# google-research/seed_rl

Hardware: NVIDIA H100
Metric: env-frames/sec (learner, device-timed) on synthetic 84x84x4 T=20 unrolls @1/2/4/8 H100 (higher is better)
Workload: dtype bf16x3 (fp32-faithful tensor-core contraction; activations stored as bf16 hi+lo pairs), f32 elsewhere

## Files before the change

### seed_rl_b200/csrc/conv_planes.cu

```cuda
#include <cuda.h>
#include <cuda_bf16.h>

#include <cstdio>
#include <cstdlib>

#include "kernels.h"
#include "tc_common.cuh"

namespace seedrl {

long long planes_positions(int N, int H, int W) {
  const long long Q = (long long)N * (H + 1) * (W + 2);
  return ((Q + 2 * (W + 2) + 2 + 256 + 127) / 128) * 128;
}
size_t planes_bytes(int N, int H, int W, int C) {
  return (size_t)planes_positions(N, H, W) * 16 * 2 * (C / 8);
}

typedef CUresult (*EncodeTiledFn)(CUtensorMap*, CUtensorMapDataType, cuuint32_t, void*, const cuuint64_t*,
                                  const cuuint64_t*, const cuuint32_t*, const cuuint32_t*,
                                  CUtensorMapInterleave, CUtensorMapSwizzle, CUtensorMapL2promotion,
                                  CUtensorMapFloatOOBfill);
static EncodeTiledFn encode_tiled_fn() {
  static EncodeTiledFn fn = nullptr;
  static bool tried = false;
  if (!tried) {
    tried = true;
    void* q = nullptr;
    cudaDriverEntryPointQueryResult qr;
    if (cudaGetDriverEntryPoint("cuTensorMapEncodeTiled", &q, cudaEnableDefault, &qr) == cudaSuccess &&
        qr == cudaDriverEntryPointSuccess)
      fn = reinterpret_cast<EncodeTiledFn>(q);
    (void)cudaGetLastError();
  }
  return fn;
}

static int g_chunk = 0;
int planes_chunk() {
  if (g_chunk == 0) {
    const char* e = getenv("SEEDRL_PLANES_CHUNK");
    g_chunk = e ? atoi(e) : 128;
    if (g_chunk != 16 && g_chunk != 32 && g_chunk != 64 && g_chunk != 128) g_chunk = 128;
  }
  return g_chunk;
}

static int make_plane_map(CUtensorMap* tm, const void* base, long long Lp, int planes, int shift,
                          int CH, int box_chunks, int box_planes) {
  EncodeTiledFn enc = encode_tiled_fn();
  if (!enc) return set_error(SEEDRL_ERR_INTERNAL, "cuTensorMapEncodeTiled is not available");
  if (box_chunks < 1 || box_chunks > 256 || box_planes < 1 || box_planes > planes)
    return set_error(SEEDRL_ERR_INVALID_ARGUMENT, "conv planes: TMA box out of range");
  const cuuint64_t gdim[3] = {(cuuint64_t)(2 * CH), (cuuint64_t)((Lp - shift) / CH), (cuuint64_t)planes};
  const cuuint64_t gstr[2] = {(cuuint64_t)CH * 16, (cuuint64_t)Lp * 16};
  const cuuint32_t box[3] = {(cuuint32_t)(2 * CH), (cuuint32_t)box_chunks, (cuuint32_t)box_planes};
  const cuuint32_t estr[3] = {1, 1, 1};
  void* addr = const_cast<char*>(reinterpret_cast<const char*>(base)) + (size_t)shift * 16;
  const CUresult r = enc(tm, CU_TENSOR_MAP_DATA_TYPE_UINT64, 3, addr, gdim, gstr, box, estr,
                         CU_TENSOR_MAP_INTERLEAVE_NONE, CU_TENSOR_MAP_SWIZZLE_NONE,
                         CU_TENSOR_MAP_L2_PROMOTION_L2_256B, CU_TENSOR_MAP_FLOAT_OOB_FILL_NONE);
  if (r != CUDA_SUCCESS) {
    char msg[128];
    snprintf(msg, sizeof msg, "cuTensorMapEncodeTiled failed (%d) Lp=%lld planes=%d shift=%d box=%dx%d", (int)r, Lp,
             planes, shift, box_chunks, box_planes);
    return set_error(SEEDRL_ERR_INTERNAL, msg);
  }
  return SEEDRL_OK;
}

__device__ __forceinline__ void mbar_expect_tx(uint64_t* bar, uint32_t bytes) {
  asm volatile("mbarrier.arrive.expect_tx.shared::cta.b64 _, [%0], %1;" ::"r"(smem_u32(bar)), "r"(bytes)
               : "memory");
}
__device__ __forceinline__ void tma_load_3d(void* dst, const CUtensorMap* tm, int c0, int c1, int c2,
                                            uint64_t* bar) {
  asm volatile(
      "cp.async.bulk.tensor.3d.shared::cluster.global.tile.mbarrier::complete_tx::bytes [%0], [%1, {%2, %3, %4}], [%5];" ::
          "r"(smem_u32(dst)),
      "l"(reinterpret_cast<uint64_t>(tm)), "r"(c0), "r"(c1), "r"(c2), "r"(smem_u32(bar))
      : "memory");
}
__device__ __forceinline__ float bf16lo(uint32_t w) { return __uint_as_float(w << 16); }
__device__ __forceinline__ float bf16hi(uint32_t w) { return __uint_as_float(w & 0xFFFF0000u); }

struct ConvpArgs {
  ConvGeom g;
  int Lp;
  int nch;
  int chunk;
  int ntiles;
  int nb;
  const uint4* wq;
  const float* bias;
  const uint4* mask;
  const uint4* res;
  uint4* out_raw;
  uint4* out_relu;
  float* out_nhwc;
  int* err;
};

constexpr int kCpWarpgroups = 4;
constexpr int kCpThreads = 128 * kCpWarpgroups + 32;
constexpr int kCpM = 128;
constexpr int kCpMaxStages = 4;

__device__ __forceinline__ void quad_transpose(float2 (&t)[4], int q) {
#pragma unroll
  for (int b = 1; b <= 2; b <<= 1) {
    const bool up = (q & b) != 0;
#pragma unroll
    for (int u = 0; u < 4; ++u) {
      if (u & b) continue;
      const float2 send = up ? t[u] : t[u | b];
      const float2 r = make_float2(__shfl_xor_sync(0xffffffffu, send.x, b), __shfl_xor_sync(0xffffffffu, send.y, b));
      if (up) t[u] = r; else t[u | b] = r;
    }
  }
}

template <int CIN, int COUT, int NSUB>
__global__ void __launch_bounds__(kCpThreads, 1)
convp_kernel(const __grid_constant__ CUtensorMap tm_in, const ConvpArgs a) {
  constexpr int G = CIN / 8, GO = COUT / 8, NS = CIN / 16;
  constexpr int MT = NSUB * kCpM;
  constexpr int NBLK = 2 * NSUB;
  extern __shared__ __align__(128) uint8_t smem_raw[];
  const int PW = a.g.PW, nb = a.nb;
  const uint32_t P = (uint32_t)(a.nch * a.chunk) * 16u;
  const uint32_t stage_bytes = 2u * G * P;
  uint8_t* s_stage = smem_raw;
  uint4* s_b = reinterpret_cast<uint4*>(smem_raw + (size_t)nb * stage_bytes);
  float* s_bias = reinterpret_cast<float*>(s_b + 2 * 9 * CIN * COUT / 8);
  uint64_t* s_full = reinterpret_cast<uint64_t*>(s_bias + COUT);
  uint64_t* s_empty = s_full + kCpMaxStages;
  const int tid = threadIdx.x, warp = tid >> 5, lane = tid & 31;

  for (int i = tid; i < 2 * 9 * CIN * COUT / 8; i += kCpThreads) s_b[i] = __ldg(a.wq + i);
  if (tid < COUT) s_bias[tid] = a.bias ? __ldg(a.bias + tid) : 0.f;
  if (tid == 0) {
    for (int i = 0; i < nb; ++i) {
      mbar_init(s_full + i, 1);
      mbar_init(s_empty + i, 4 * kCpWarpgroups);
    }
    asm volatile("fence.mbarrier_init.release.cluster;" ::: "memory");
    asm volatile("prefetch.tensormap [%0];" ::"l"(reinterpret_cast<uint64_t>(&tm_in)) : "memory");
  }
  asm volatile("fence.proxy.async.shared::cta;" ::: "memory");
  __syncthreads();

  const int my_tiles = ((int)blockIdx.x < a.ntiles) ? (a.ntiles - 1 - (int)blockIdx.x) / (int)gridDim.x + 1 : 0;
  bool timed_out = false;

  if (warp == 4 * kCpWarpgroups) {
    if (elect_one()) {
      for (int it = 0; it < my_tiles; ++it) {
        const int s = it % nb;
        if (it >= nb && !mbar_wait_bounded(s_empty + s, (uint32_t)(((it / nb) - 1) & 1))) { timed_out = true; break; }
        const int tile = (int)blockIdx.x + it * (int)gridDim.x;
        mbar_expect_tx(s_full + s, stage_bytes);
        tma_load_3d(s_stage + (size_t)s * stage_bytes, &tm_in, 0, tile * MT / a.chunk, 0, s_full + s);
      }
    }
    __syncwarp();
  } else {
    const int cw = warp >> 2;
    const size_t plane_u = (size_t)a.Lp;
    if (blockIdx.x == 0) {
      const uint4 z = make_uint4(0u, 0u, 0u, 0u);
      for (int i = tid; i < (PW + 1) * 2 * GO; i += 128 * kCpWarpgroups) {
        const int pl = i / (PW + 1), s = i - pl * (PW + 1);
        if (a.out_raw) a.out_raw[(size_t)pl * plane_u + s] = z;
        if (a.out_relu) a.out_relu[(size_t)pl * plane_u + s] = z;
      }
    }
    const int q = lane & 3;
    const int row = 16 * (warp & 3) + (lane >> 2) + 8 * (q & 1);
    const uint32_t b_base = smem_u32(s_b);
    const uint64_t db0 = gmma_desc(b_base, (uint32_t)(2 * GO) * 128u, 128u);
    for (int it = 0; it < my_tiles; ++it) {
      const int s = it % nb;
      const int tile = (int)blockIdx.x + it * (int)gridDim.x;
      if (!mbar_wait_bounded(s_full + s, (uint32_t)((it / nb) & 1))) { timed_out = true; break; }
      const int m0 = (cw - it * NBLK) & (kCpWarpgroups - 1);
      if (m0 >= NBLK && lane == 0) mbar_arrive(s_empty + s);
      const uint32_t a_base = smem_u32(s_stage + (size_t)s * stage_bytes);
      const uint64_t da0 = gmma_desc(a_base, P, 128u);
      const uint64_t lo_off = (uint64_t)((G * P) >> 4), slab_off = (uint64_t)((2 * P) >> 4);
#pragma unroll 1
      for (int m = m0; m < NBLK; m += kCpWarpgroups) {
        float acc[COUT];
#pragma unroll
        for (int i = 0; i < COUT; ++i) acc[i] = 0.f;
        wgmma_fence_acc<COUT>(acc);
        wgmma_fence();
#pragma unroll
        for (int tap = 0; tap < 9; ++tap) {
          const uint64_t off = (uint64_t)(m * 64 + (tap / 3) * PW + (tap % 3));
#pragma unroll
          for (int sl = 0; sl < NS; ++sl) {
            const uint64_t da = da0 + off + (uint64_t)sl * slab_off;
            const uint64_t db = db0 + (uint64_t)((tap * NS + sl) * (COUT * 64 / 16));
            Wgmma<2 * COUT>::template mma<0, 0>(acc, da, db, 1u);
            Wgmma<COUT>::template mma<0, 0>(acc, da + lo_off, db, 1u);
          }
        }
        wgmma_commit();
        const int p = tile * MT + m * 64 + row;
        const int sp = p + PW + 1;
        const int pix = out_pixel(a.g, p);
        uint4 mk[GO / 2], rh[GO / 2], rl[GO / 2];
        if (pix >= 0) {
#pragma unroll
          for (int k = 0; k < GO / 2; ++k) {
            const int go = (q >> 1) + 2 * k;
            if (a.mask) mk[k] = __ldg(a.mask + (size_t)go * plane_u + sp);
            if (a.res) {
              rh[k] = __ldg(a.res + (size_t)go * plane_u + sp);
              rl[k] = __ldg(a.res + (size_t)(GO + go) * plane_u + sp);
            }
          }
        }
        wgmma_wait<0>();
        wgmma_fence_acc<COUT>(acc);
        if (m + kCpWarpgroups >= NBLK && lane == 0) mbar_arrive(s_empty + s);
        const bool in_store = sp < a.Lp;
#pragma unroll
        for (int k = 0; k < GO / 2; ++k) {
          const int go = (q >> 1) + 2 * k;
          float2 t[4];
#pragma unroll
          for (int u = 0; u < 4; ++u) {
            const int j = 2 * k + (u >> 1), h = u & 1;
            t[u] = make_float2(acc[4 * j + 2 * h] + acc[4 * (j + GO) + 2 * h],
                               acc[4 * j + 2 * h + 1] + acc[4 * (j + GO) + 2 * h + 1]);
          }
          quad_transpose(t, q);
          float x[8];
#pragma unroll
          for (int e = 0; e < 4; ++e) {
            x[2 * e] = t[e].x + s_bias[go * 8 + 2 * e];
            x[2 * e + 1] = t[e].y + s_bias[go * 8 + 2 * e + 1];
          }
          if (pix >= 0 && a.mask) {
            const uint32_t mw[4] = {mk[k].x, mk[k].y, mk[k].z, mk[k].w};
#pragma unroll
            for (int e = 0; e < 4; ++e) {
              x[2 * e] = bf16lo(mw[e]) > 0.f ? x[2 * e] : 0.f;
              x[2 * e + 1] = bf16hi(mw[e]) > 0.f ? x[2 * e + 1] : 0.f;
            }
          }
          if (pix >= 0 && a.res) {
            const uint32_t hw[4] = {rh[k].x, rh[k].y, rh[k].z, rh[k].w};
            const uint32_t lw[4] = {rl[k].x, rl[k].y, rl[k].z, rl[k].w};
#pragma unroll
            for (int e = 0; e < 4; ++e) {
              x[2 * e] += bf16lo(hw[e]) + bf16lo(lw[e]);
              x[2 * e + 1] += bf16hi(hw[e]) + bf16hi(lw[e]);
            }
          }
          if (pix < 0) {
#pragma unroll
            for (int e = 0; e < 8; ++e) x[e] = 0.f;
          }
          const float4 xa = make_float4(x[0], x[1], x[2], x[3]), xb = make_float4(x[4], x[5], x[6], x[7]);
          if (a.out_raw && in_store) {
            a.out_raw[(size_t)go * plane_u + sp] = pack8_bf16(xa, xb);
            a.out_raw[(size_t)(GO + go) * plane_u + sp] = pack8_bf16(bf16_resid4(xa), bf16_resid4(xb));
          }
          if (a.out_relu && in_store) {
            const float4 ra = make_float4(fmaxf(xa.x, 0.f), fmaxf(xa.y, 0.f), fmaxf(xa.z, 0.f), fmaxf(xa.w, 0.f));
            const float4 rb = make_float4(fmaxf(xb.x, 0.f), fmaxf(xb.y, 0.f), fmaxf(xb.z, 0.f), fmaxf(xb.w, 0.f));
            a.out_relu[(size_t)go * plane_u + sp] = pack8_bf16(ra, rb);
            a.out_relu[(size_t)(GO + go) * plane_u + sp] = pack8_bf16(bf16_resid4(ra), bf16_resid4(rb));
          }
          if (a.out_nhwc && pix >= 0) {
            float4* o = reinterpret_cast<float4*>(a.out_nhwc + (size_t)pix * COUT + go * 8);
            o[0] = xa; o[1] = xb;
          }
        }
      }
    }
  }
  if (timed_out && a.err) atomicExch(a.err, 1);
}

template <int CIN, int COUT, int NSUB>
static int launch_convp(const PlaneConv& c, cudaStream_t st) {
  const ConvGeom g = make_geom(c.N, c.H, c.W);
  constexpr int MT = NSUB * kCpM;
  const long long Lp = planes_positions(c.N, c.H, c.W);
  if (Lp + MT + 4 * g.PW >= (1LL << 31))
    return set_error(SEEDRL_ERR_INVALID_ARGUMENT, "convp: batch too large for 32-bit positions");
  const int L = MT + 2 * g.PW + 2;
  const int CH = planes_chunk();
  const int nch = (L + CH - 1) / CH;
  const size_t stage = (size_t)2 * (CIN / 8) * nch * CH * 16;
  const size_t fixed = (size_t)2 * 9 * CIN * COUT * 2 + COUT * 4 + 2 * kCpMaxStages * 8;
  int nb = kCpMaxStages;
  while (nb > 1 && nb * stage + fixed > 227 * 1024) --nb;
  if (nb < 2) return kPlanesTryNext;
  const size_t smem = nb * stage + fixed;
  CUtensorMap tm;
  SEEDRL_TRY(make_plane_map(&tm, c.in, Lp, 2 * (CIN / 8), 0, CH, nch, 2 * (CIN / 8)));
  static bool attr = false;
  if (!attr) {
    SEEDRL_CUDA(cudaFuncSetAttribute(convp_kernel<CIN, COUT, NSUB>, cudaFuncAttributeMaxDynamicSharedMemorySize,
                                     227 * 1024));
    attr = true;
  }
  ConvpArgs a;
  a.g = g; a.Lp = (int)Lp; a.nch = nch; a.chunk = CH; a.nb = nb;
  a.ntiles = (int)((Lp - g.PW - 1 + MT - 1) / MT);
  a.wq = reinterpret_cast<const uint4*>(c.wq); a.bias = c.bias;
  a.mask = reinterpret_cast<const uint4*>(c.mask); a.res = reinterpret_cast<const uint4*>(c.res);
  a.out_raw = reinterpret_cast<uint4*>(c.out_raw); a.out_relu = reinterpret_cast<uint4*>(c.out_relu);
  a.out_nhwc = c.out_nhwc; a.err = c.err;
  const int grid = a.ntiles < kNumSMs ? a.ntiles : kNumSMs;
  convp_kernel<CIN, COUT, NSUB><<<grid, kCpThreads, smem, st>>>(tm, a);
  count_launch(g_conv_cat, st);
  SEEDRL_CHECK_LAUNCH();
  return SEEDRL_OK;
}

bool convp_supported(int cin, int cout) {
  return (cin == 16 || cin == 32) && (cout == 16 || cout == 32);
}

int convp_forward(int cin, int cout, const PlaneConv& c, cudaStream_t st) {
  const long long Lp = planes_positions(c.N, c.H, c.W);
  const bool small = Lp / 512 < 2 * kNumSMs;
#define SEEDRL_CP_CASE(CI, CO_)                                                   \
  if (cin == CI && cout == CO_) {                                                 \
    int rc = kPlanesTryNext;                                                      \
    if (!small) rc = launch_convp<CI, CO_, 4>(c, st);                             \
    if (rc == kPlanesTryNext) rc = launch_convp<CI, CO_, 2>(c, st);               \
    if (rc == kPlanesTryNext) rc = launch_convp<CI, CO_, 1>(c, st);               \
    if (rc == kPlanesTryNext) return set_error(SEEDRL_ERR_INVALID_ARGUMENT, "convp: image too wide"); \
    return rc;                                                                    \
  }
  SEEDRL_CP_CASE(16, 16)
  SEEDRL_CP_CASE(16, 32)
  SEEDRL_CP_CASE(32, 16)
  SEEDRL_CP_CASE(32, 32)
#undef SEEDRL_CP_CASE
  return set_error(SEEDRL_ERR_INVALID_ARGUMENT, "convp: unsupported (cin,cout)");
}

struct WgradpArgs {
  int PW, T, nchunks, nb;
  int chunk;
  float* partial;
  int* err;
};

constexpr int kWpMaxStages = 6;
constexpr int kWpHaloRow = 8;
__host__ __device__ constexpr int wgradp_mtiles(int CP) { return 3 * CP + 1 <= 64 ? 1 : 2; }
__host__ __device__ constexpr int wgradp_khsplit(int CP) { return CP == 16 ? 3 : 1; }
__host__ __device__ constexpr int wgradp_threads(int CP) { return 128 * wgradp_mtiles(CP) * wgradp_khsplit(CP) + 32; }

struct WgradMaps { CUtensorMap x, x_halo, dy, dy_halo; };

template <int CP, int COUT, int KC>
__global__ void __launch_bounds__(wgradp_threads(CP), 1)
wgradp_kernel(const __grid_constant__ WgradMaps tm, const WgradpArgs a) {
  constexpr int G = CP / 8, GO = COUT / 8;
  constexpr int MT = wgradp_mtiles(CP), KSPL = wgradp_khsplit(CP), NCW = MT * KSPL;
  constexpr int NKH = 3 / KSPL;
  constexpr int NW = 9 * CP * COUT + COUT;
  constexpr uint32_t Px = (KC + kWpHaloRow) * 16;
  extern __shared__ __align__(128) uint8_t smem_raw[];
  const int nb = a.nb, PW = a.PW;
  const uint32_t Pd = (uint32_t)(KC + a.T) * 16u;
  const uint32_t x_bytes = 2u * G * Px;
  const uint32_t stage_bytes = x_bytes + 2u * GO * Pd;
  uint64_t* s_full = reinterpret_cast<uint64_t*>(smem_raw);
  uint64_t* s_empty = s_full + kWpMaxStages;
  uint8_t* s_stage = smem_raw + 128;
  const int tid = threadIdx.x, warp = tid >> 5, lane = tid & 31;

  if (tid == 0) {
    for (int i = 0; i < kWpMaxStages; ++i) { mbar_init(s_full + i, 1); mbar_init(s_empty + i, 4 * NCW); }
    asm volatile("fence.mbarrier_init.release.cluster;" ::: "memory");
  }
  __syncthreads();

  const int my_chunks = ((int)blockIdx.x < a.nchunks) ? (a.nchunks - 1 - (int)blockIdx.x) / (int)gridDim.x + 1 : 0;
  bool timed_out = false;

  if (warp == 4 * NCW) {
    if (elect_one()) {
      for (int it = 0; it < my_chunks; ++it) {
        const int s = it % nb;
        if (it >= nb && !mbar_wait_bounded(s_empty + s, (uint32_t)(((it / nb) - 1) & 1))) { timed_out = true; break; }
        const int j0 = ((int)blockIdx.x + it * (int)gridDim.x) * KC;
        uint8_t* xs = s_stage + (size_t)s * stage_bytes;
        uint8_t* ds = xs + x_bytes;
        mbar_expect_tx(s_full + s, stage_bytes);
        for (int p = 0; p < 2 * G; ++p) {
          tma_load_3d(xs + p * Px, &tm.x, 0, j0 / a.chunk, p, s_full + s);
          tma_load_3d(xs + p * Px + KC * 16, &tm.x_halo, 0, (j0 + KC) / kWpHaloRow, p, s_full + s);
        }
        for (int p = 0; p < 2 * GO; ++p) {
          tma_load_3d(ds + p * Pd, &tm.dy, 0, j0 / a.chunk, p, s_full + s);
          tma_load_3d(ds + p * Pd + KC * 16, &tm.dy_halo, 0, (j0 + KC) / kWpHaloRow, p, s_full + s);
        }
      }
    }
    __syncwarp();
  } else {
    const int cw = warp >> 2, mt = cw % MT, kh0 = (cw / MT) * NKH;
    const int mg0 = 8 * mt + 2 * (warp & 3);
    const int mg = mg0 + ((lane >> 3) & 1);
    const uint32_t a_off = (mg < 3 * G ? (uint32_t)(mg % G) * Px + (uint32_t)(mg / G) * 16u : 0u) +
                           (uint32_t)((lane >> 4) * 8 + (lane & 7)) * 16u;
    const bool data0 = mg0 < 3 * G, data1 = mg0 + 1 < 3 * G;
    const uint32_t one = (lane >> 2) == 0 ? 0x3F803F80u : 0u;
    const uint32_t c0 = mg0 == 3 * G ? one : 0u, c1 = mg0 + 1 == 3 * G ? one : 0u;
    float acc[NKH][COUT];
#pragma unroll
    for (int i = 0; i < NKH * COUT; ++i) (&acc[0][0])[i] = 0.f;
    wgmma_fence_acc<NKH * COUT>(&acc[0][0]);
    const uint64_t desc0 = gmma_desc(0u, 128u, Pd);
    const uint32_t desc_lo = (uint32_t)desc0, desc_hi = (uint32_t)(desc0 >> 32);
    for (int it = 0; it < my_chunks; ++it) {
      const int s = it % nb;
      if (!mbar_wait_bounded(s_full + s, (uint32_t)((it / nb) & 1))) { timed_out = true; break; }
      const uint32_t sb = smem_u32(s_stage + (size_t)s * stage_bytes);
      const uint32_t xb = sb + a_off;
      const uint32_t db = desc_lo + ((sb + x_bytes) >> 4) + (uint32_t)((2 - kh0) * PW);
      uint32_t ah[2][4], al[2][4];
#pragma unroll
      for (int ks = 0; ks < KC / 16; ++ks) {
        uint32_t(&h)[4] = ah[ks & 1];
        uint32_t(&l)[4] = al[ks & 1];
        ldsm_x4_trans(h, xb + ks * 256);
        ldsm_x4_trans(l, xb + G * Px + ks * 256);
        if (!data0) { h[0] = h[2] = c0; l[0] = l[2] = 0u; }
        if (!data1) { h[1] = h[3] = c1; l[1] = l[3] = 0u; }
        wgmma_fence();
#pragma unroll
        for (int kh = 0; kh < NKH; ++kh) {
          const uint64_t b = make_desc64(db - (uint32_t)(kh * PW) + (uint32_t)(ks * 16), desc_hi);
          WgmmaRA<2 * COUT>::template mma<1>(acc[kh], h, b, 1u);
          WgmmaRA<COUT>::template mma<1>(acc[kh], l, b, 1u);
        }
        wgmma_commit();
        wgmma_wait<1>();
      }
      wgmma_wait<0>();
      if (lane == 0) mbar_arrive(s_empty + s);
    }
    wgmma_fence_acc<NKH * COUT>(&acc[0][0]);
    float* dst = a.partial + (size_t)blockIdx.x * NW;
#pragma unroll
    for (int h = 0; h < 2; ++h) {
      const int row = 64 * mt + 16 * (warp & 3) + (lane >> 2) + 8 * h;
      const int kw = row / CP, ci = row - kw * CP;
#pragma unroll
      for (int k = 0; k < NKH; ++k) {
        const int kh = kh0 + k;
#pragma unroll
        for (int j = 0; j < GO; ++j) {
#pragma unroll
          for (int e = 0; e < 2; ++e) {
            const int co = 8 * j + 2 * (lane & 3) + e;
            const float v = acc[k][4 * j + 2 * h + e] + acc[k][4 * j + 2 * h + e + COUT / 2];
            if (row < 3 * CP) dst[((size_t)(kh * 3 + kw) * CP + ci) * COUT + co] = v;
            else if (row == 3 * CP && kh == 1) dst[9 * CP * COUT + co] = v;
          }
        }
      }
    }
  }
  if (timed_out && a.err) atomicExch(a.err, 1);
}

template <int CP, int COUT, int KC>
static int launch_wgradp(int N, int H, int W, const void* x, const void* dy, float* dw, float* db, int* err,
                         WgradBatch* batch, cudaStream_t st) {
  const ConvGeom g = make_geom(N, H, W);
  const long long Lp = planes_positions(N, H, W);
  constexpr int G = CP / 8, GO = COUT / 8;
  const int CH = planes_chunk() < KC ? planes_chunk() : KC;
  if (KC % CH) return kPlanesTryNext;
  const int T = (2 * g.PW + kWpHaloRow - 1) / kWpHaloRow * kWpHaloRow;
  const size_t stage = (size_t)2 * G * (KC + kWpHaloRow) * 16 + (size_t)2 * GO * (KC + T) * 16;
  int nb = kWpMaxStages;
  while (nb > 1 && 128 + nb * stage > 227 * 1024) --nb;
  if (nb < 2) return kPlanesTryNext;
  const size_t smem = 128 + nb * stage;
  WgradMaps tm;
  SEEDRL_TRY(make_plane_map(&tm.x, x, Lp, 2 * G, g.PW, CH, KC / CH, 1));
  SEEDRL_TRY(make_plane_map(&tm.x_halo, x, Lp, 2 * G, g.PW, kWpHaloRow, 1, 1));
  SEEDRL_TRY(make_plane_map(&tm.dy, dy, Lp, 2 * GO, 1, CH, KC / CH, 1));
  SEEDRL_TRY(make_plane_map(&tm.dy_halo, dy, Lp, 2 * GO, 1, kWpHaloRow, T / kWpHaloRow, 1));
  static bool attr = false;
  if (!attr) {
    SEEDRL_CUDA(cudaFuncSetAttribute(wgradp_kernel<CP, COUT, KC>, cudaFuncAttributeMaxDynamicSharedMemorySize,
                                     227 * 1024));
    attr = true;
  }
  static const bool dbg = getenv("SEEDRL_DEBUG_LAUNCH") != nullptr;
  if (dbg) fprintf(stderr, "wgradp<%d,%d,%d> CH=%d T=%d nb=%d stage=%zu smem=%zu\n", CP, COUT, KC, CH, T, nb, stage, smem);
  constexpr int NW = 9 * CP * COUT + COUT;
  WgradpArgs a;
  a.PW = g.PW; a.T = T; a.nb = nb; a.err = err; a.chunk = CH;
  a.nchunks = (int)((g.Q + g.PW + KC - 1) / KC);
  const int grid = a.nchunks < kNumSMs ? a.nchunks : kNumSMs;
  if (!batch || batch->n >= kMaxReduceJobs || batch->used + (size_t)grid * NW > batch->cap_floats)
    return set_error(SEEDRL_ERR_INVALID_ARGUMENT, "wgradp: partial buffer too small");
  a.partial = batch->buf + batch->used;
  batch->used += (size_t)grid * NW;
  wgradp_kernel<CP, COUT, KC><<<grid, wgradp_threads(CP), smem, st>>>(tm, a);
  count_launch(PC_CONV_WGRAD, st);
  SEEDRL_CHECK_LAUNCH();
  batch->jobs[batch->n++] = ReduceJob{a.partial, dw, db, grid, 9 * CP * COUT, COUT};
  return SEEDRL_OK;
}

int wgradp(int cin, int cout, int N, int H, int W, const void* x, const void* dy, float* dw, float* db,
           int* err, WgradBatch* batch, cudaStream_t st) {
#define SEEDRL_WP_CASE(CI, CO_, KC0)                                                                        \
  if (cin == CI && cout == CO_) {                                                                           \
    int rc = kPlanesTryNext;                                                                                \
    if constexpr (KC0 >= 256) rc = launch_wgradp<CI, CO_, 256>(N, H, W, x, dy, dw, db, err, batch, st);     \
    if (rc == kPlanesTryNext) rc = launch_wgradp<CI, CO_, 128>(N, H, W, x, dy, dw, db, err, batch, st);     \
    if (rc == kPlanesTryNext) rc = launch_wgradp<CI, CO_, 64>(N, H, W, x, dy, dw, db, err, batch, st);      \
    if (rc == kPlanesTryNext) return set_error(SEEDRL_ERR_INVALID_ARGUMENT, "wgradp: does not fit");        \
    return rc;                                                                                              \
  }
  SEEDRL_WP_CASE(16, 16, 256)
  SEEDRL_WP_CASE(16, 32, 128)
  SEEDRL_WP_CASE(32, 32, 128)
#undef SEEDRL_WP_CASE
  return set_error(SEEDRL_ERR_INVALID_ARGUMENT, "wgradp: unsupported (cin,cout)");
}

__global__ void to_planes_kernel(ConvGeom g, int Lp, int G, int relu, const float* __restrict__ x,
                                 uint4* __restrict__ out) {
  const long long i = (long long)blockIdx.x * blockDim.x + threadIdx.x;
  if (i >= (long long)Lp * G) return;
  const int s = (int)(i / G), go = (int)(i - (long long)s * G);
  const int pix = in_pixel(g, s);
  float4 a = make_float4(0.f, 0.f, 0.f, 0.f), b = a;
  if (pix >= 0) {
    const float4* src = reinterpret_cast<const float4*>(x + (size_t)pix * (G * 8) + go * 8);
    a = __ldg(src); b = __ldg(src + 1);
    if (relu) {
      a.x = fmaxf(a.x, 0.f); a.y = fmaxf(a.y, 0.f); a.z = fmaxf(a.z, 0.f); a.w = fmaxf(a.w, 0.f);
      b.x = fmaxf(b.x, 0.f); b.y = fmaxf(b.y, 0.f); b.z = fmaxf(b.z, 0.f); b.w = fmaxf(b.w, 0.f);
    }
  }
  out[(size_t)go * Lp + s] = pack8_bf16(a, b);
  out[(size_t)(G + go) * Lp + s] = pack8_bf16(bf16_resid4(a), bf16_resid4(b));
}

__global__ void from_planes_kernel(ConvGeom g, int Lp, int G, const uint4* __restrict__ in, float* __restrict__ y) {
  const long long i = (long long)blockIdx.x * blockDim.x + threadIdx.x;
  if (i >= (long long)Lp * G) return;
  const int s = (int)(i / G), go = (int)(i - (long long)s * G);
  const int pix = in_pixel(g, s);
  if (pix < 0) return;
  const uint4 h = __ldg(in + (size_t)go * Lp + s), l = __ldg(in + (size_t)(G + go) * Lp + s);
  float4* dst = reinterpret_cast<float4*>(y + (size_t)pix * (G * 8) + go * 8);
  dst[0] = make_float4(bf16lo(h.x) + bf16lo(l.x), bf16hi(h.x) + bf16hi(l.x), bf16lo(h.y) + bf16lo(l.y),
                       bf16hi(h.y) + bf16hi(l.y));
  dst[1] = make_float4(bf16lo(h.z) + bf16lo(l.z), bf16hi(h.z) + bf16hi(l.z), bf16lo(h.w) + bf16lo(l.w),
                       bf16hi(h.w) + bf16hi(l.w));
}

int to_planes(int N, int H, int W, int C, int relu, const float* x, void* out, cudaStream_t st) {
  const ConvGeom g = make_geom(N, H, W);
  const long long Lp = planes_positions(N, H, W);
  const long long n = Lp * (C / 8);
  to_planes_kernel<<<(unsigned)((n + 255) / 256), 256, 0, st>>>(g, (int)Lp, C / 8, relu, x,
                                                                reinterpret_cast<uint4*>(out));
  count_launch(PC_MISC, st);
  SEEDRL_CHECK_LAUNCH();
  return SEEDRL_OK;
}
int from_planes(int N, int H, int W, int C, const void* in, float* y, cudaStream_t st) {
  const ConvGeom g = make_geom(N, H, W);
  const long long Lp = planes_positions(N, H, W);
  const long long n = Lp * (C / 8);
  from_planes_kernel<<<(unsigned)((n + 255) / 256), 256, 0, st>>>(g, (int)Lp, C / 8,
                                                                  reinterpret_cast<const uint4*>(in), y);
  count_launch(PC_MISC, st);
  SEEDRL_CHECK_LAUNCH();
  return SEEDRL_OK;
}

__global__ void poolp_fwd_kernel(ConvGeom go_, int Lp, int G, int H, int W, int pt, int pl,
                                 const float* __restrict__ x, uint4* __restrict__ out_raw,
                                 uint4* __restrict__ out_relu, uint8_t* __restrict__ idx) {
  const long long i = (long long)blockIdx.x * blockDim.x + threadIdx.x;
  if (i >= (long long)Lp * G) return;
  const int s = (int)(i / G), gq = (int)(i - (long long)s * G);
  const int pix = in_pixel(go_, s);
  float best[8];
  unsigned char arg[8];
#pragma unroll
  for (int e = 0; e < 8; ++e) { best[e] = 0.f; arg[e] = 0; }
  if (pix >= 0) {
    const int Wo = go_.W, Ho = go_.H, C = G * 8;
    const int n = pix / (Ho * Wo), r = pix - n * (Ho * Wo), ho = r / Wo, wo = r - ho * Wo;
#pragma unroll
    for (int e = 0; e < 8; ++e) best[e] = -INFINITY;
#pragma unroll
    for (int kh = 0; kh < 3; ++kh) {
      const int h = ho * 2 - pt + kh;
      if (h < 0 || h >= H) continue;
#pragma unroll
      for (int kw = 0; kw < 3; ++kw) {
        const int w = wo * 2 - pl + kw;
        if (w < 0 || w >= W) continue;
        const float4* src = reinterpret_cast<const float4*>(x + ((size_t)(n * H + h) * W + w) * C + gq * 8);
        const float4 a = __ldg(src), b = __ldg(src + 1);
        const float v[8] = {a.x, a.y, a.z, a.w, b.x, b.y, b.z, b.w};
        const unsigned char t = (unsigned char)(kh * 3 + kw);
#pragma unroll
        for (int e = 0; e < 8; ++e)
          if (v[e] > best[e]) { best[e] = v[e]; arg[e] = t; }
      }
    }
    uint2 packed;
    packed.x = arg[0] | (arg[1] << 8) | (arg[2] << 16) | ((uint32_t)arg[3] << 24);
    packed.y = arg[4] | (arg[5] << 8) | (arg[6] << 16) | ((uint32_t)arg[7] << 24);
    *reinterpret_cast<uint2*>(idx + (size_t)pix * C + gq * 8) = packed;
  }
  const float4 a = make_float4(best[0], best[1], best[2], best[3]), b = make_float4(best[4], best[5], best[6], best[7]);
  out_raw[(size_t)gq * Lp + s] = pack8_bf16(a, b);
  out_raw[(size_t)(G + gq) * Lp + s] = pack8_bf16(bf16_resid4(a), bf16_resid4(b));
  const float4 ra = make_float4(fmaxf(a.x, 0.f), fmaxf(a.y, 0.f), fmaxf(a.z, 0.f), fmaxf(a.w, 0.f));
  const float4 rb = make_float4(fmaxf(b.x, 0.f), fmaxf(b.y, 0.f), fmaxf(b.z, 0.f), fmaxf(b.w, 0.f));
  out_relu[(size_t)gq * Lp + s] = pack8_bf16(ra, rb);
  out_relu[(size_t)(G + gq) * Lp + s] = pack8_bf16(bf16_resid4(ra), bf16_resid4(rb));
}

template <bool OUT_PLANES>
__global__ void poolp_bwd_kernel(ConvGeom gf, int Lpf, ConvGeom gp, int Lpp, int G, int pt, int pl,
                                 const uint4* __restrict__ dy, const uint8_t* __restrict__ idx,
                                 uint4* __restrict__ dx_planes, float* __restrict__ dx_nhwc) {
  const long long i = (long long)blockIdx.x * blockDim.x + threadIdx.x;
  const int H = gf.H, W = gf.W, Ho = gp.H, Wo = gp.W, C = G * 8;
  int gq, s = 0, pix;
  if (OUT_PLANES) {
    if (i >= (long long)Lpf * G) return;
    s = (int)(i / G); gq = (int)(i - (long long)s * G);
    pix = in_pixel(gf, s);
  } else {
    if (i >= (long long)gf.N * H * W * G) return;
    pix = (int)(i / G); gq = (int)(i - (long long)pix * G);
  }
  float acc[8];
#pragma unroll
  for (int e = 0; e < 8; ++e) acc[e] = 0.f;
  if (pix >= 0) {
    const int n = pix / (H * W), r = pix - n * (H * W), h = r / W, w = r - h * W;
    const int hp = h + pt, wp = w + pl;
#pragma unroll
    for (int dh = 0; dh < 2; ++dh) {
      const int ho = (hp >> 1) - dh;
      const int kh = hp - 2 * ho;
      if (ho < 0 || ho >= Ho || kh > 2) continue;
#pragma unroll
      for (int dw = 0; dw < 2; ++dw) {
        const int wo = (wp >> 1) - dw;
        const int kw = wp - 2 * wo;
        if (wo < 0 || wo >= Wo || kw > 2) continue;
        const unsigned tap = (unsigned)(kh * 3 + kw);
        const size_t o = ((size_t)(n * Ho + ho) * Wo + wo) * C + gq * 8;
        const uint2 t = __ldg(reinterpret_cast<const uint2*>(idx + o));
        const int sp = (n * gp.RH + ho + 1) * gp.PW + wo + 1;
        const uint4 hh = __ldg(dy + (size_t)gq * Lpp + sp), ll = __ldg(dy + (size_t)(G + gq) * Lpp + sp);
        const float gv[8] = {bf16lo(hh.x) + bf16lo(ll.x), bf16hi(hh.x) + bf16hi(ll.x), bf16lo(hh.y) + bf16lo(ll.y),
                             bf16hi(hh.y) + bf16hi(ll.y), bf16lo(hh.z) + bf16lo(ll.z), bf16hi(hh.z) + bf16hi(ll.z),
                             bf16lo(hh.w) + bf16lo(ll.w), bf16hi(hh.w) + bf16hi(ll.w)};
#pragma unroll
        for (int e = 0; e < 8; ++e) {
          const unsigned te = ((e < 4 ? t.x : t.y) >> (8 * (e & 3))) & 0xFFu;
          if (te == tap) acc[e] += gv[e];
        }
      }
    }
  }
  const float4 a = make_float4(acc[0], acc[1], acc[2], acc[3]), b = make_float4(acc[4], acc[5], acc[6], acc[7]);
  if (OUT_PLANES) {
    dx_planes[(size_t)gq * Lpf + s] = pack8_bf16(a, b);
    dx_planes[(size_t)(G + gq) * Lpf + s] = pack8_bf16(bf16_resid4(a), bf16_resid4(b));
  } else {
    float4* dst = reinterpret_cast<float4*>(dx_nhwc + (size_t)pix * C + gq * 8);
    dst[0] = a; dst[1] = b;
  }
}

static void same_pad3s2(int in, int* out, int* before) {
  *out = (in + 1) / 2;
  const int total = (*out - 1) * 2 + 3 - in;
  *before = total > 0 ? total / 2 : 0;
}

int poolp_forward(int N, int H, int W, int C, const float* x, void* out_raw, void* out_relu, uint8_t* idx,
                  cudaStream_t st) {
  int Ho, Wo, pt, pl;
  same_pad3s2(H, &Ho, &pt);
  same_pad3s2(W, &Wo, &pl);
  const ConvGeom g = make_geom(N, Ho, Wo);
  const long long Lp = planes_positions(N, Ho, Wo);
  const long long n = Lp * (C / 8);
  poolp_fwd_kernel<<<(unsigned)((n + 255) / 256), 256, 0, st>>>(g, (int)Lp, C / 8, H, W, pt, pl, x,
                                                                reinterpret_cast<uint4*>(out_raw),
                                                                reinterpret_cast<uint4*>(out_relu), idx);
  count_launch(PC_POOL, st);
  SEEDRL_CHECK_LAUNCH();
  return SEEDRL_OK;
}

int poolp_backward(int N, int H, int W, int C, const void* dy, const uint8_t* idx, void* dx_planes,
                   float* dx_nhwc, cudaStream_t st) {
  int Ho, Wo, pt, pl;
  same_pad3s2(H, &Ho, &pt);
  same_pad3s2(W, &Wo, &pl);
  const ConvGeom gf = make_geom(N, H, W), gp = make_geom(N, Ho, Wo);
  const long long Lpf = planes_positions(N, H, W), Lpp = planes_positions(N, Ho, Wo);
  if (dx_planes) {
    const long long n = Lpf * (C / 8);
    poolp_bwd_kernel<true><<<(unsigned)((n + 255) / 256), 256, 0, st>>>(
        gf, (int)Lpf, gp, (int)Lpp, C / 8, pt, pl, reinterpret_cast<const uint4*>(dy), idx,
        reinterpret_cast<uint4*>(dx_planes), nullptr);
  } else {
    const long long n = (long long)N * H * W * (C / 8);
    poolp_bwd_kernel<false><<<(unsigned)((n + 255) / 256), 256, 0, st>>>(
        gf, (int)Lpf, gp, (int)Lpp, C / 8, pt, pl, reinterpret_cast<const uint4*>(dy), idx, nullptr, dx_nhwc);
  }
  count_launch(PC_POOL, st);
  SEEDRL_CHECK_LAUNCH();
  return SEEDRL_OK;
}

}
```

Before: 198,500.

## Prefetch residual and mask operands via TMA ring in plane conv kernel

Adds a second producer lane that uses TMA to stream the residual (hi/lo) and mask planes for each tile into a two-slot shared-memory ring, guarded by its own full/empty mbarriers. Consumer warpgroups then read these operands from shared memory instead of issuing per-thread __ldg gathers in the epilogue. The path is used only when mask or residual is present and no relu output is requested. The goal is to overlap epilogue operand fetches with the MMA main loop. The ring costs extra shared memory, which may reduce the number of input pipeline stages, and adds barrier synchronisation plus more tensor maps.

```diff
diff --git a/seed_rl_b200/csrc/conv_planes.cu b/seed_rl_b200/csrc/conv_planes.cu
--- a/seed_rl_b200/csrc/conv_planes.cu
+++ b/seed_rl_b200/csrc/conv_planes.cu
@@ -3,6 +3,7 @@
 
 #include <cstdio>
 #include <cstdlib>
+#include <cstring>
 
 #include "kernels.h"
 #include "tc_common.cuh"
@@ -105,6 +106,9 @@
 constexpr int kCpThreads = 128 * kCpWarpgroups + 32;
 constexpr int kCpM = 128;
 constexpr int kCpMaxStages = 4;
+constexpr int kCpOpSlots = 2;
+
+struct ConvpMaps { CUtensorMap in, res, mask; };
 
 __device__ __forceinline__ void quad_transpose(float2 (&t)[4], int q) {
 #pragma unroll
@@ -120,9 +124,9 @@
   }
 }
 
-template <int CIN, int COUT, int NSUB>
+template <int CIN, int COUT, int NSUB, bool RING>
 __global__ void __launch_bounds__(kCpThreads, 1)
-convp_kernel(const __grid_constant__ CUtensorMap tm_in, const ConvpArgs a) {
+convp_kernel(const __grid_constant__ ConvpMaps tm, const ConvpArgs a) {
   constexpr int G = CIN / 8, GO = COUT / 8, NS = CIN / 16;
   constexpr int MT = NSUB * kCpM;
   constexpr int NBLK = 2 * NSUB;
@@ -130,11 +134,16 @@
   const int PW = a.g.PW, nb = a.nb;
   const uint32_t P = (uint32_t)(a.nch * a.chunk) * 16u;
   const uint32_t stage_bytes = 2u * G * P;
+  const int res_planes = a.res ? 2 * GO : 0;
+  const uint32_t op_bytes = RING ? (uint32_t)(res_planes + (a.mask ? GO : 0)) * MT * 16u : 0u;
   uint8_t* s_stage = smem_raw;
-  uint4* s_b = reinterpret_cast<uint4*>(smem_raw + (size_t)nb * stage_bytes);
+  uint8_t* s_ops = smem_raw + (size_t)nb * stage_bytes;
+  uint4* s_b = reinterpret_cast<uint4*>(s_ops + (RING ? kCpOpSlots : 0) * op_bytes);
   float* s_bias = reinterpret_cast<float*>(s_b + 2 * 9 * CIN * COUT / 8);
   uint64_t* s_full = reinterpret_cast<uint64_t*>(s_bias + COUT);
   uint64_t* s_empty = s_full + kCpMaxStages;
+  uint64_t* s_ofull = s_empty + kCpMaxStages;
+  uint64_t* s_oempty = s_ofull + kCpOpSlots;
   const int tid = threadIdx.x, warp = tid >> 5, lane = tid & 31;
 
   for (int i = tid; i < 2 * 9 * CIN * COUT / 8; i += kCpThreads) s_b[i] = __ldg(a.wq + i);
@@ -144,8 +153,14 @@
       mbar_init(s_full + i, 1);
       mbar_init(s_empty + i, 4 * kCpWarpgroups);
     }
+    if (RING) {
+      for (int i = 0; i < kCpOpSlots; ++i) {
+        mbar_init(s_ofull + i, 1);
+        mbar_init(s_oempty + i, 4 * kCpWarpgroups);
+      }
+    }
     asm volatile("fence.mbarrier_init.release.cluster;" ::: "memory");
-    asm volatile("prefetch.tensormap [%0];" ::"l"(reinterpret_cast<uint64_t>(&tm_in)) : "memory");
+    asm volatile("prefetch.tensormap [%0];" ::"l"(reinterpret_cast<uint64_t>(&tm.in)) : "memory");
   }
   asm volatile("fence.proxy.async.shared::cta;" ::: "memory");
   __syncthreads();
@@ -154,13 +169,26 @@
   bool timed_out = false;
 
   if (warp == 4 * kCpWarpgroups) {
-    if (elect_one()) {
+    if (lane == 0) {
       for (int it = 0; it < my_tiles; ++it) {
         const int s = it % nb;
         if (it >= nb && !mbar_wait_bounded(s_empty + s, (uint32_t)(((it / nb) - 1) & 1))) { timed_out = true; break; }
         const int tile = (int)blockIdx.x + it * (int)gridDim.x;
         mbar_expect_tx(s_full + s, stage_bytes);
-        tma_load_3d(s_stage + (size_t)s * stage_bytes, &tm_in, 0, tile * MT / a.chunk, 0, s_full + s);
+        tma_load_3d(s_stage + (size_t)s * stage_bytes, &tm.in, 0, tile * MT / a.chunk, 0, s_full + s);
+      }
+    } else if (RING && lane == 1) {
+      for (int it = 0; it < my_tiles; ++it) {
+        const int o = it % kCpOpSlots;
+        if (it >= kCpOpSlots && !mbar_wait_bounded(s_oempty + o, (uint32_t)(((it / kCpOpSlots) - 1) & 1))) {
+          timed_out = true;
+          break;
+        }
+        const int c = ((int)blockIdx.x + it * (int)gridDim.x) * MT / a.chunk;
+        uint8_t* slot = s_ops + (size_t)o * op_bytes;
+        mbar_expect_tx(s_ofull + o, op_bytes);
+        if (a.res) tma_load_3d(slot, &tm.res, 0, c, 0, s_ofull + o);
+        if (a.mask) tma_load_3d(slot + (size_t)res_planes * MT * 16, &tm.mask, 0, c, 0, s_ofull + o);
       }
     }
     __syncwarp();
@@ -184,7 +212,16 @@
       const int tile = (int)blockIdx.x + it * (int)gridDim.x;
       if (!mbar_wait_bounded(s_full + s, (uint32_t)((it / nb) & 1))) { timed_out = true; break; }
       const int m0 = (cw - it * NBLK) & (kCpWarpgroups - 1);
-      if (m0 >= NBLK && lane == 0) mbar_arrive(s_empty + s);
+      const int oslot = it % kCpOpSlots;
+      const uint32_t ophase = (uint32_t)((it / kCpOpSlots) & 1);
+      if (m0 >= NBLK) {
+        if (RING && !mbar_wait_bounded(s_ofull + oslot, ophase)) { timed_out = true; break; }
+        if (lane == 0) {
+          mbar_arrive(s_empty + s);
+          if (RING) mbar_arrive(s_oempty + oslot);
+        }
+      }
+      const uint4* s_op = reinterpret_cast<const uint4*>(s_ops + (size_t)oslot * op_bytes);
       const uint32_t a_base = smem_u32(s_stage + (size_t)s * stage_bytes);
       const uint64_t da0 = gmma_desc(a_base, P, 128u);
       const uint64_t lo_off = (uint64_t)((G * P) >> 4), slab_off = (uint64_t)((2 * P) >> 4);
@@ -211,7 +248,23 @@
         const int sp = p + PW + 1;
         const int pix = out_pixel(a.g, p);
         uint4 mk[GO / 2], rh[GO / 2], rl[GO / 2];
-        if (pix >= 0) {
+        if (RING) {
+          if (m == m0 && !mbar_wait_bounded(s_ofull + oslot, ophase)) {
+            wgmma_wait<0>();
+            timed_out = true;
+            break;
+          }
+          const int lp = m * 64 + row;
+#pragma unroll
+          for (int k = 0; k < GO / 2; ++k) {
+            const int go = (q >> 1) + 2 * k;
+            if (a.mask) mk[k] = s_op[(res_planes + go) * MT + lp];
+            if (a.res) {
+              rh[k] = s_op[go * MT + lp];
+              rl[k] = s_op[(GO + go) * MT + lp];
+            }
+          }
+        } else if (pix >= 0) {
 #pragma unroll
           for (int k = 0; k < GO / 2; ++k) {
             const int go = (q >> 1) + 2 * k;
@@ -280,16 +333,21 @@
             o[0] = xa; o[1] = xb;
           }
         }
-      }
+        if (RING && m + kCpWarpgroups >= NBLK) {
+          __syncwarp();
+          if (lane == 0) mbar_arrive(s_oempty + oslot);
+        }
+      }
+      if (timed_out) break;
     }
   }
   if (timed_out && a.err) atomicExch(a.err, 1);
 }
 
-template <int CIN, int COUT, int NSUB>
+template <int CIN, int COUT, int NSUB, bool RING>
 static int launch_convp(const PlaneConv& c, cudaStream_t st) {
   const ConvGeom g = make_geom(c.N, c.H, c.W);
-  constexpr int MT = NSUB * kCpM;
+  constexpr int MT = NSUB * kCpM, GO = COUT / 8;
   const long long Lp = planes_positions(c.N, c.H, c.W);
   if (Lp + MT + 4 * g.PW >= (1LL << 31))
     return set_error(SEEDRL_ERR_INVALID_ARGUMENT, "convp: batch too large for 32-bit positions");
@@ -297,19 +355,27 @@
   const int CH = planes_chunk();
   const int nch = (L + CH - 1) / CH;
   const size_t stage = (size_t)2 * (CIN / 8) * nch * CH * 16;
-  const size_t fixed = (size_t)2 * 9 * CIN * COUT * 2 + COUT * 4 + 2 * kCpMaxStages * 8;
+  const size_t op_slot = (size_t)((c.res ? 2 * GO : 0) + (c.mask ? GO : 0)) * MT * 16;
+  const size_t fixed = (RING ? kCpOpSlots * op_slot : 0) + (size_t)2 * 9 * CIN * COUT * 2 + COUT * 4 +
+                       (2 * kCpMaxStages + 2 * kCpOpSlots) * 8;
   int nb = kCpMaxStages;
   while (nb > 1 && nb * stage + fixed > 227 * 1024) --nb;
   if (nb < 2) return kPlanesTryNext;
   const size_t smem = nb * stage + fixed;
-  CUtensorMap tm;
-  SEEDRL_TRY(make_plane_map(&tm, c.in, Lp, 2 * (CIN / 8), 0, CH, nch, 2 * (CIN / 8)));
+  ConvpMaps tm;
+  memset(&tm, 0, sizeof tm);
+  SEEDRL_TRY(make_plane_map(&tm.in, c.in, Lp, 2 * (CIN / 8), 0, CH, nch, 2 * (CIN / 8)));
+  if (RING && c.res) SEEDRL_TRY(make_plane_map(&tm.res, c.res, Lp, 2 * GO, g.PW + 1, CH, MT / CH, 2 * GO));
+  if (RING && c.mask) SEEDRL_TRY(make_plane_map(&tm.mask, c.mask, Lp, GO, g.PW + 1, CH, MT / CH, GO));
   static bool attr = false;
   if (!attr) {
-    SEEDRL_CUDA(cudaFuncSetAttribute(convp_kernel<CIN, COUT, NSUB>, cudaFuncAttributeMaxDynamicSharedMemorySize,
-                                     227 * 1024));
+    SEEDRL_CUDA(cudaFuncSetAttribute(convp_kernel<CIN, COUT, NSUB, RING>,
+                                     cudaFuncAttributeMaxDynamicSharedMemorySize, 227 * 1024));
     attr = true;
   }
+  static const bool dbg = getenv("SEEDRL_DEBUG_LAUNCH") != nullptr;
+  if (dbg) fprintf(stderr, "convp<%d,%d,%d,%d> nb=%d stage=%zu op_slot=%zu smem=%zu\n", CIN, COUT, NSUB, (int)RING, nb,
+                   stage, op_slot, smem);
   ConvpArgs a;
   a.g = g; a.Lp = (int)Lp; a.nch = nch; a.chunk = CH; a.nb = nb;
   a.ntiles = (int)((Lp - g.PW - 1 + MT - 1) / MT);
@@ -318,10 +384,16 @@
   a.out_raw = reinterpret_cast<uint4*>(c.out_raw); a.out_relu = reinterpret_cast<uint4*>(c.out_relu);
   a.out_nhwc = c.out_nhwc; a.err = c.err;
   const int grid = a.ntiles < kNumSMs ? a.ntiles : kNumSMs;
-  convp_kernel<CIN, COUT, NSUB><<<grid, kCpThreads, smem, st>>>(tm, a);
+  convp_kernel<CIN, COUT, NSUB, RING><<<grid, kCpThreads, smem, st>>>(tm, a);
   count_launch(g_conv_cat, st);
   SEEDRL_CHECK_LAUNCH();
   return SEEDRL_OK;
+}
+
+template <int CIN, int COUT, int NSUB>
+static int launch_convp(const PlaneConv& c, cudaStream_t st) {
+  const bool ring = (c.mask || c.res) && !c.out_relu;
+  return ring ? launch_convp<CIN, COUT, NSUB, true>(c, st) : launch_convp<CIN, COUT, NSUB, false>(c, st);
 }
 
 bool convp_supported(int cin, int cout) {
```

Result: no change. 200,400, median of 6 (+1.0%).
